# addtt/ladder-vae-pytorch

Hardware: AMD Instinct MI355X
Metric: training images/sec (ELBO step: fwd+bwd+Adamax) (higher is better)
Workload: dtype f32; 1 GPU; CIFAR10-shaped 15-layer LVAE (BASELINE configs[2]): 32x32x3, zdims 32x15, 4 blocks/layer, 64 filters, gated+skip, DMoL-10, dropout 0.2, free bits 1.0; batch_per_gpu=256, global_batch=256, parallelism=dp1, hip_graph=True

## Files before the change

### include/lvae_hip.h

```cpp
#ifndef LVAE_HIP_H
#define LVAE_HIP_H

#include <stddef.h>
#include <stdint.h>

#ifdef __cplusplus
extern "C" {
#endif

#define LVAE_ABI_VERSION 17

#define LVAE_EINVAL (-1)
#define LVAE_EALIGN (-2)
#define LVAE_EWORKSPACE (-3)

enum { LVAE_STATS_BN_FWD = 0, LVAE_STATS_BN_BWD = 1 };
enum { LVAE_PREC_F32 = 0, LVAE_PREC_BF16 = 1 };
enum { LVAE_DT_F32 = 0, LVAE_DT_BF16 = 1 };
enum {
  LVAE_FORM_AUTO = 0,
  LVAE_FORM_F32_MFMA = 1,
  LVAE_FORM_SIX_PRODUCT = 2,
  LVAE_FORM_SIX_PRODUCT_DIRECT = 3
};
// ... 96 lines not shown
  const float* dh;
  const float* x;
  const float* add;
  float* dgamma;
  float* dbeta;
  float* out;
  int32_t dh_bf16;
  int32_t reserved_;
  const float* drop;
} lvae_bn_apply;
size_t lvae_conv1x1_gate_bwd_wgrad_workspace(const lvae_conv_desc* d);
int32_t lvae_conv1x1_gate_bwd_wgrad_apply_ok(const lvae_conv_desc* d);
int lvae_conv1x1_gate_bwd_wgrad_f32(const lvae_conv_desc* d, const float* dout, const float* ab, const float* y, int32_t act,
                                    float* dw, int64_t dw_sk, int64_t dw_sn, float* db, void* workspace, size_t workspace_bytes,
                                    const lvae_bn_apply* ap, void* stream);

enum { LVAE_RB_PRO_AFFINE = 0, LVAE_RB_PRO_BN_APPLY = 1, LVAE_RB_PRO_GATE_BWD = 2 };
enum { LVAE_RB_EPI_PLAIN = 0, LVAE_RB_EPI_GATE = 1 };
typedef struct lvae_rb_ext {
  int32_t prologue, epilogue;
  const float* gate_w;
  int64_t gate_w_sk, gate_w_sn;
  void* gate_ws;
  int64_t gate_ws_bytes;
  int32_t gate_ws_ready;
  const float* gate_bias;
  int32_t act;
  const float* res;
  float* ab;
  float* out;
// ... 286 lines not shown
```

### ladder-vae-pytorch_amd/_C.py

```python
import ctypes as C
import os

import torch

_HERE = os.path.dirname(os.path.abspath(__file__))
LIB_PATH = os.path.join(_HERE, 'liblvae_hip.so')

ACT = {None: 0, 'none': 0, 'elu': 1, 'relu': 2, 'leakyrelu': 3, 'selu': 4}
GATHER_CONV, GATHER_TRANSPOSED = 0, 1
PREC_F32, PREC_BF16 = 0, 1
DT_F32, DT_BF16 = 0, 1
VARIANT_DIRECT, VARIANT_POS, VARIANT_WINO_F32, VARIANT_WINO_SIX, VARIANT_BF16_DIRECT, VARIANT_SIX_DIRECT = 0, 2, 3, 4, 5, 6
GATE_PERSISTENT, GATE_SINGLE_SHOT = 1, 2
WGRAD_VARIANT_GENERIC, WGRAD_VARIANT_IMG, WGRAD_VARIANT_BF16, WGRAD_VARIANT_WINO, WGRAD_VARIANT_DIRECT_1X1, WGRAD_VARIANT_TILE, WGRAD_VARIANT_THIN = range(7)
FEED_U8, FEED_F32 = 0, 1
FORM_AUTO, FORM_F32_MFMA, FORM_SIX_PRODUCT, FORM_SIX_PRODUCT_DIRECT = 0, 1, 2, 3


class LvaeHipError(RuntimeError):
    pass


class ConvDesc(C.Structure):
    _fields_ = [
# ... 82 lines not shown
    'lvae_conv2d_position_major': (_I, [C.POINTER(ConvDesc)]),
    'lvae_resblock_bf16_storage': (_I, [C.POINTER(ConvDesc)]),
    'lvae_conv2d_folds_bn_finalize': (_I, [C.POINTER(ConvDesc)]),
    'lvae_conv2d_stats_buffer_rows': (_I, [C.POINTER(ConvDesc)]),
    'lvae_conv2d_prepare_entry_bytes': (_Z, []),
    'lvae_conv2d_prepare_entry': (C.c_int, [C.POINTER(ConvDesc), _P]),
    'lvae_conv2d_prepare_weights': (C.c_int, [_P, _I, _I, _P]),
    'lvae_conv1x1_gate_f32': (C.c_int, [C.POINTER(ConvDesc), _P, _I, _P, _P]),
    'lvae_conv1x1_gate_stats_rows': (_I, [C.POINTER(ConvDesc)]),
    'lvae_conv1x1_gate_variant': (_I, [C.POINTER(ConvDesc)]),
    'lvae_conv1x1_gate_bwd_f32': (C.c_int, [C.POINTER(ConvDesc), _P, _P, _I, _P, _P]),
    'lvae_conv1x1_gate_bwd_ok': (_I, [C.POINTER(ConvDesc)]),
    'lvae_conv1x1_gate_bwd_wgrad_workspace': (_Z, [C.POINTER(ConvDesc)]),
    'lvae_conv1x1_gate_bwd_wgrad_apply_ok': (_I, [C.POINTER(ConvDesc)]),
    'lvae_conv1x1_gate_bwd_wgrad_f32': (C.c_int, [C.POINTER(ConvDesc), _P, _P, _P, _I, _P, _L, _L, _P, _P, _Z, C.POINTER(BnApply), _P]),
    'lvae_resblock_gate_workspace': (_Z, [C.POINTER(ConvDesc)]),
    'lvae_resblock_gate_prepare_entry': (C.c_int, [C.POINTER(ConvDesc), _P]),
    'lvae_resblock_conv_rows': (_I, [C.POINTER(ConvDesc)]),
    'lvae_resblock_conv_gate_rows': (_I, [C.POINTER(ConvDesc)]),
    'lvae_resblock_conv_workspace': (_Z, [C.POINTER(ConvDesc)]),
    'lvae_resblock_conv_prepare_entry': (C.c_int, [C.POINTER(ConvDesc), _P]),
    'lvae_resblock_conv_f32': (C.c_int, [C.POINTER(ConvDesc), C.POINTER(RbExt), _P]),
    'lvae_conv2d_wgrad_workspace': (_Z, [C.POINTER(ConvDesc)]),
    'lvae_conv2d_wgrad_f32': (C.c_int, [C.POINTER(ConvDesc), _P, _P, _P, _P, _Z, _P]),
    'lvae_conv2d_wgrad_bf16': (C.c_int, [C.POINTER(ConvDesc), _P, _P, _P, _P, _Z, _P]),
    'lvae_conv2d_wgrad_variant': (_I, [C.POINTER(ConvDesc)]),
    'lvae_conv2d_wgrad_apply_ok': (_I, [C.POINTER(ConvDesc)]),
    'lvae_conv2d_wgrad_apply_f32': (C.c_int, [C.POINTER(ConvDesc), C.POINTER(BnApply), _P, _P, _P, _Z, _P]),
    'lvae_conv2d_wgrad_pair_ok': (_I, [C.POINTER(ConvDesc), C.POINTER(ConvDesc)]),
    'lvae_conv2d_wgrad_pair_workspace': (_Z, [C.POINTER(ConvDesc), C.POINTER(ConvDesc)]),
# ... 141 lines not shown
```

### ladder-vae-pytorch_amd/csrc/conv1x1_gate_bwd_fused.hip

```cpp
#include "bf16_frag.h"
#include "bn_stats.h"
#include "lvae_host.h"

namespace lvae {

struct GbfArgs {
  const float* dout;
  const float* ab;
  const float* y;
  const float* w;
  int64_t w_sn;
  const float* drop;
  float* dx;
  float* slab_w;
  float* slab_b;
  int M, ohw, ntiles, act;
  int in_bf16, dx_bf16;
  lvae_bn_apply ap;
};

constexpr int GB_LDA = 132;
constexpr int GB_LDY = 68;

__global__ __launch_bounds__(512) void conv1x1_gate_bwd_fused_kernel(GbfArgs a) {
  kernarg_warmup<(sizeof(GbfArgs) < 1024 ? sizeof(GbfArgs) : 1024)>();
  extern __shared__ __attribute__((aligned(16))) float smem[];
  float* Bs = smem;
  float* As = Bs + 64 * GB_LDA;
  float* Ys = As + 64 * GB_LDA;
  const int t = threadIdx.x, lane = t & 63, wave = t >> 6;
  const bool wg_role = wave >= 4;
  const int wm = (wave & 3) >> 1, wn = wave & 1, li = lane & 31, lh = lane >> 5;
  const f32x4 zero4 = {0.f, 0.f, 0.f, 0.f};
// ... 110 lines not shown
    if (t < 128) {
      float v = 0.f;
#pragma unroll
      for (int g = 0; g < 32; ++g) v += red[g * 128 + t];
      a.slab_b[(size_t)blockIdx.x * 128 + t] = v;
    }
  }
}

constexpr int GBB_LDA = 136;
constexpr int GBB_LDY = 72;
constexpr size_t gbb_lds(int split) {
  return (size_t)split * (64 * GBB_LDA + 64 * GBB_LDY) * 2 + (size_t)64 * GB_LDY * 4 + 6 * 64 * 4 + (split == 3 ? (size_t)8 * 2 * 3 * 64 * 16 : 0);
}

template <int SPLIT, bool S16 = false, bool AP = false, bool ELU = false>
__global__ __launch_bounds__(512) void conv1x1_gate_bwd_fused_bf16_kernel(GbfArgs a) {
  kernarg_warmup<sizeof(GbfArgs)>();
#ifdef LVAE_GBF_DBG
  constexpr int dbg = LVAE_GBF_DBG;
#else
  constexpr int dbg = 0;
#endif
  const int gact = ELU ? LVAE_ACT_ELU : a.act, apact = ELU ? LVAE_ACT_ELU : a.ap.act;
  static_assert(SPLIT == 1 || !S16, "bf16 storage exists for the bf16-operand form only");
  extern __shared__ __attribute__((aligned(16))) unsigned char smem_raw[];
  constexpr int A_PLANE = 64 * GBB_LDA, Y_PLANE = 64 * GBB_LDY;
  __bf16* As = reinterpret_cast<__bf16*>(smem_raw);
  __bf16* Ys = As + SPLIT * A_PLANE;
  float* Os = reinterpret_cast<float*>(Ys + SPLIT * Y_PLANE);
  float* Cf = Os + 64 * GB_LDY;
  const int t = threadIdx.x, lane = t & 63, wave = t >> 6;
  const bool wg_role = wave >= 4;
  const int wm = (wave & 3) >> 1, wn = wave & 1, li = lane & 31, lh = lane >> 5, G = lane >> 4, i16 = lane & 15;
  const f32x4 zero4 = {0.f, 0.f, 0.f, 0.f};

  if (AP) {
    const int q = t & 31, rg = t >> 5, rows = a.ap.rows;
    f32x4 acc = zero4;
    for (int r = rg; r < rows; r += 16 * 8) {
// ... 65 lines not shown
  auto prefetch_row = [&](int tile, int u) {
    if (dbg & 1) {
      pg[u] = pa[u] = pb[u] = py[u] = zero4;
      if (AP) px[u] = pd[u] = zero4;
      return;
    }
    const int m = tile * 64 + r0 + 32 * u;
    const size_t mc = m < a.M ? (size_t)m : 0;
    if (AP) {
      pg[u] = load4_dt(a.ap.dh, mc * 64 + c4, ap_dh_bf);
      px[u] = *reinterpret_cast<const f32x4*>(a.ap.x + mc * 64 + c4);
      pd[u] = ap_add ? *reinterpret_cast<const f32x4*>(a.ap.add + mc * 64 + c4) : zero4;
    } else {
      pg[u] = *reinterpret_cast<const f32x4*>(a.dout + mc * 64 + c4);
    }
    pa[u] = load4_dt(a.ab, mc * 128 + c4, a.in_bf16 != 0);
    pb[u] = load4_dt(a.ab, mc * 128 + 64 + c4, a.in_bf16 != 0);
    py[u] = load4_dt(a.y, mc * 64 + c4, a.in_bf16 != 0);
  };
  auto prefetch = [&](int tile) {
    const int m0 = tile * 64;
    if (dbg & 1) {
      pg[0] = pg[1] = zero4;
#pragma unroll
      for (int u = 0; u < IT; ++u) pa[u] = pb[u] = py[u] = zero4;
#pragma unroll
      for (int u = 0; u < (AP ? 2 : 1); ++u) px[u] = pd[u] = zero4;
      qa = qb = qy = bf16x8{0, 0, 0, 0, 0, 0, 0, 0};
      return;
    }
    if (S16) {
      const int m = m0 + r8;
// ... 16 lines not shown
    }
#pragma unroll
    for (int u = 0; u < IT; ++u) prefetch_row(tile, u);
  };

  f32x16 accw[2];
#pragma unroll
  for (int j = 0; j < 2; ++j)
#pragma unroll
    for (int r = 0; r < 16; ++r) accw[j][r] = 0.f;
  f32x4 bs_lo = zero4, bs_hi = zero4;
  f32x4 bs_lo8 = zero4, bs_hi8 = zero4;
  const int trow = 8 * (G >> 1) + (i16 >> 2), tch = 16 * (G & 1) + 4 * (i16 & 3);
  using PO = PieceOrder<SPLIT>;

  int tile = blockIdx.x;
  if (tile < a.ntiles) prefetch(tile);
  for (; tile < a.ntiles; tile += gridDim.x) {
    const int m0 = tile * 64;
    if (S16) {
      f32x4 lo[2] = {zero4, zero4}, hi[2] = {zero4, zero4};
      bf16x8 yv = {0, 0, 0, 0, 0, 0, 0, 0};
      if (m0 + r8 < a.M) {
        if (AP) {
#pragma unroll
          for (int h = 0; h < 2; ++h) {
            pg[h] = ap_value(pg[h], px[h], pd[h], c8 + 4 * h);
            store_wt4(a.ap.out + (size_t)(m0 + r8) * 64 + c8 + 4 * h, pg[h]);
          }
        }
// ... 3 lines not shown
          for (int j = 0; j < 4; ++j) {
            const float av = (float)qa[4 * h + j], bv = (float)qb[4 * h + j];
            const float sg = sigmoidf_(bv);
            lo[h][j] = pg[h][j] * sg * act_grad(av, gact);
            hi[h][j] = pg[h][j] * act_fwd(av, gact) * sg * (1.f - sg);
          }
        yv = qy;
      }
      bs_lo += lo[0];
      bs_lo8 += lo[1];
      bs_hi += hi[0];
      bs_hi8 += hi[1];
      *reinterpret_cast<bf16x8*>(As + r8 * GBB_LDA + c8) = to_bf16x8(lo[0], lo[1]);
      *reinterpret_cast<bf16x8*>(As + r8 * GBB_LDA + 64 + c8) = to_bf16x8(hi[0], hi[1]);
      *reinterpret_cast<bf16x8*>(Ys + r8 * GBB_LDY + c8) = yv;
    } else
#pragma unroll
    for (int u = 0; u < IT; ++u) {
      const int r = r0 + 32 * u;
      f32x4 lo = zero4, hi = zero4, yv = zero4;
      if (m0 + r < a.M) {
        if (AP) {
          pg[u] = ap_value(pg[u], px[u], pd[u], c4);
          if (!(dbg & 4)) store_wt4(a.ap.out + (size_t)(m0 + r) * 64 + c4, pg[u]);
        }
        if (dbg & 8) {
          lo = pg[u] + pa[u];
          hi = pg[u] + pb[u];
        } else
#pragma unroll
        for (int j = 0; j < 4; ++j) {
// ... 2 lines not shown
          hi[j] = pg[u][j] * act_fwd(pa[u][j], gact) * sg * (1.f - sg);
        }
        yv = py[u];
      }
      bs_lo += lo;
      bs_hi += hi;
      if (tile + (int)gridDim.x < a.ntiles) prefetch_row(tile + gridDim.x, u);
      bf16x4 pl[SPLIT], ph[SPLIT], pyv[SPLIT];
      split4<SPLIT>(lo, pl);
      split4<SPLIT>(hi, ph);
      split4<SPLIT>(yv, pyv);
#pragma unroll
      for (int q = 0; q < SPLIT; ++q) {
        *reinterpret_cast<bf16x4*>(As + q * A_PLANE + r * GBB_LDA + c4) = pl[q];
        *reinterpret_cast<bf16x4*>(As + q * A_PLANE + r * GBB_LDA + 64 + c4) = ph[q];
        *reinterpret_cast<bf16x4*>(Ys + q * Y_PLANE + r * GBB_LDY + c4) = pyv[q];
      }
    }
    if (S16 && tile + (int)gridDim.x < a.ntiles) prefetch(tile + gridDim.x);
    lds_barrier();

    if (!wg_role) {
      f32x16 accx;
#pragma unroll
      for (int r = 0; r < 16; ++r) accx[r] = 0.f;
#pragma unroll
      for (int s = 0; s < 8; ++s) {
        bf16x8 af[SPLIT];
#pragma unroll
        for (int q = 0; q < SPLIT; ++q)
          af[q] = *reinterpret_cast<const bf16x8*>(As + q * A_PLANE + (wm * 32 + li) * GBB_LDA + 16 * s + 8 * lh);
        if (WLDS) {
// ... 103 lines not shown
  if (off || d == nullptr) return false;
  if (d->KH != 1 || d->KW != 1 || d->stride != 1 || d->pad != 0 || d->OH != d->H || d->OW != d->W) return false;
  if (d->C1 != 128 || d->C2 != 0 || d->Cout != 64 || d->w_sk != 1 || d->w_sn % 4 != 0 || d->in_scale != nullptr) return false;
  if (!al16_or_null(d->w) || !al16_or_null(d->y) || !al16_or_null(d->out_scale)) return false;
  const bool bf16 = d->precision == LVAE_PREC_BF16;
  if ((d->x_dtype == LVAE_DT_BF16 || d->y_dtype == LVAE_DT_BF16) && !bf16) return false;
  if (with_apply && d->form == LVAE_FORM_F32_MFMA && !bf16) return false;
  const int64_t M = (int64_t)d->N * d->H * d->W;
  static const int64_t min_m = tune("LVAE_GATE_FUSED_MIN_M", 256 * 64);
  if (M < min_m || M >= ((int64_t)1 << 31)) return false;
  p = ConvPlan{};
  p.workspace = (size_t)gbf_nwg(M) * (64 * 128 + 128) * sizeof(float);
  return true;
}

#define GBF_REQUIRE_AL16(p) LVAE_REQUIRE(al16_or_null(p), LVAE_EALIGN, "lvae_conv1x1_gate_bwd_wgrad_f32: " #p " must be 16-byte aligned")

static int conv1x1_gate_bwd_fused_launch(const lvae_conv_desc* d, const float* dout, const float* ab, const float* y, int act, float* dw,
                                         int64_t dw_sk, int64_t dw_sn, float* db, void* workspace, const lvae_bn_apply* ap, hipStream_t s) {
  GBF_REQUIRE_AL16(dout);
  GBF_REQUIRE_AL16(ab);
  GBF_REQUIRE_AL16(y);
  GBF_REQUIRE_AL16(workspace);
  GbfArgs a;
  a.ap = lvae_bn_apply{};
  if (ap != nullptr && ap->parts != nullptr) {
    GBF_REQUIRE_AL16(ap->parts);
    GBF_REQUIRE_AL16(ap->coef);
    GBF_REQUIRE_AL16(ap->dh);
    GBF_REQUIRE_AL16(ap->x);
    GBF_REQUIRE_AL16(ap->add);
    GBF_REQUIRE_AL16(ap->out);
    a.ap = *ap;
  }
  a.dout = dout;
  a.ab = ab;
  a.y = y;
  a.w = d->w;
  a.w_sn = d->w_sn;
// ... 19 lines not shown
  do {                                                                                                                                    \
    if (elu) hipLaunchKernelGGL((conv1x1_gate_bwd_fused_bf16_kernel<1, S16_, AP_, true>), grid, block, gbb_lds(1), s, a);                \
    else hipLaunchKernelGGL((conv1x1_gate_bwd_fused_bf16_kernel<1, S16_, AP_, false>), grid, block, gbb_lds(1), s, a);                   \
  } while (0)
    if (with_ap) {
      if (a.in_bf16 && a.dx_bf16) GBF_LAUNCH(true, true);
      else GBF_LAUNCH(false, true);
    } else if (a.in_bf16 && a.dx_bf16) GBF_LAUNCH(true, false);
    else GBF_LAUNCH(false, false);
#undef GBF_LAUNCH
    LVAE_LAUNCH_CHECK(name);
  } else {
    constexpr size_t lds3 = gbb_lds(3);
    int rc;
    if (f32_mfma) rc = launch_lds<conv1x1_gate_bwd_fused_kernel>(name, grid, block, lds, (int)lds, s, a);
    else if (with_ap && elu) rc = launch_lds<conv1x1_gate_bwd_fused_bf16_kernel<3, false, true, true>>(name, grid, block, lds3, (int)lds3, s, a);
    else if (with_ap) rc = launch_lds<conv1x1_gate_bwd_fused_bf16_kernel<3, false, true, false>>(name, grid, block, lds3, (int)lds3, s, a);
    else if (elu) rc = launch_lds<conv1x1_gate_bwd_fused_bf16_kernel<3, false, false, true>>(name, grid, block, lds3, (int)lds3, s, a);
    else rc = launch_lds<conv1x1_gate_bwd_fused_bf16_kernel<3, false, false, false>>(name, grid, block, lds3, (int)lds3, s, a);
    if (rc) return rc;
  }
  wgrad_reduce_launch(a.slab_w, a.slab_b, nwg, 1, 64, 128, 0, dw_sk, dw_sn, dw, db, s);
  LVAE_LAUNCH_CHECK("conv1x1_gate_bwd_fused_reduce");
  return 0;
}

}

using namespace lvae;

// ... 11 lines not shown
                                               float* dw, int64_t dw_sk, int64_t dw_sn, float* db, void* workspace,
                                               size_t workspace_bytes, const lvae_bn_apply* ap, void* stream) {
  const bool with_ap = ap != nullptr && ap->parts != nullptr;
  LVAE_REQUIRE(d && (dout || with_ap) && ab && y && d->y && dw && workspace, LVAE_EINVAL, "lvae_conv1x1_gate_bwd_wgrad_f32: null pointer");
  if (with_ap)
    LVAE_REQUIRE(ap->rows > 0 && ap->M == (int64_t)d->N * d->H * d->W && ap->coef && ap->dh && ap->x && ap->out, LVAE_EINVAL,
                 "lvae_conv1x1_gate_bwd_wgrad_f32: deferred apply needs parts / rows, M = N*H*W, the coefficient block, dh, x and out");
  ConvPlan p;
  LVAE_REQUIRE(conv1x1_gate_bwd_fused_plan(d, with_ap, p), LVAE_EINVAL,
               "lvae_conv1x1_gate_bwd_wgrad_f32: not supported (needs the gate of a 64-channel block: 1x1, 128 -> 64 dgrad view, at least 16384 "
               "pixels, 16-byte aligned w / y / out_scale, bf16 storage only with precision LVAE_PREC_BF16, a deferred apply not with "
               "LVAE_FORM_F32_MFMA); use lvae_conv1x1_gate_bwd_f32 + lvae_conv2d_wgrad_f32");
  LVAE_REQUIRE(workspace_bytes >= p.workspace, LVAE_EWORKSPACE, "lvae_conv1x1_gate_bwd_wgrad_f32: workspace %zu < %zu", workspace_bytes, p.workspace);
  return conv1x1_gate_bwd_fused_launch(d, dout, ab, y, act, dw, dw_sk, dw_sn, db, workspace, ap, (hipStream_t)stream);
}
```

### ladder-vae-pytorch_amd/kernels.py

```python
import ctypes as C
import weakref

import torch

from . import _C
from ._C import ACT, BnFold, ConvDesc, RbExt, GATHER_CONV, GATHER_TRANSPOSED, PREC_BF16, PREC_F32, call, ptr, ptr_dt, stream_ptr

_ws_cache = {}

precision = PREC_F32


form = _C.FORM_AUTO


class use_form:
    def __init__(self, f):
        self.f = f

    def __enter__(self):
        global form
        self.prev, form = form, self.f

    def __exit__(self, *exc):
# ... 317 lines not shown
    d = _desc(g, weight, ab, None, N, H, W, H, W, g.Cin, g.s_co, g.s_ci, GATHER_TRANSPOSED, out_scale=out_scale, y=dx)
    lib = _C.load()
    need = lib.lvae_conv1x1_gate_bwd_wgrad_workspace(C.byref(d))
    if not need or (apply is not None and not lib.lvae_conv1x1_gate_bwd_wgrad_apply_ok(C.byref(d))):
        return None
    ws = workspace(need, dout.device)
    ap = None
    if apply is not None:
        ap = _C.BnApply(ptr(apply.parts), apply.parts.shape[0], ACT[apply.act], N * H * W, ptr(apply.coef0), ptr_dt(apply.dh), ptr(apply.x),
                        ptr(apply.add), ptr(apply.dgamma), ptr(apply.dbeta), ptr(apply.out), int(apply.dh.dtype == torch.bfloat16), 0)
    call('lvae_conv1x1_gate_bwd_wgrad_f32', C.byref(d), ptr(dout), ptr_dt(ab), ptr_dt(y), ACT[act], ptr(dweight), g.s_ci, g.s_co, ptr(dbias),
         ws.data_ptr(), ws.numel(), C.byref(ap) if ap is not None else None, stream_ptr())
    return dx


def _rb_desc(x_like, weight, g, dgrad, y=None, bias=None, in_scale=None, in_shift=None, in_act=None, out_scale=None):
    N, H, W, _ = x_like.shape
    if dgrad:
        d = _desc(g, weight, x_like, None, N, H, W, H, W, g.Cin, g.s_co, g.s_ci, GATHER_TRANSPOSED, out_scale=out_scale, y=y)
    else:
        d = _desc(g, weight, x_like, None, N, H, W, H, W, g.Cout, g.s_ci, g.s_co, GATHER_CONV, bias, in_scale, in_shift, in_act, out_scale, None, y)
    need = _C.load().lvae_resblock_conv_workspace(C.byref(d))
    if need:
        prepared.attach(d, weight, x_like.device, need, 'lvae_resblock_conv_prepare_entry')
    return d, need


def _rb_gate_ws(e, gate_w, gate_g, device, bwd):
    gd = ConvDesc()
    gd.w, gd.precision = ptr(gate_w), precision
# ... 74 lines not shown
    return y, parts, coef


def rb_gate_rows(x, weight, g, whole_image=True):
    d = _rb_query_desc(x, weight, g)
    if d is None:
        return 0
    rows = int(_C.load().lvae_resblock_conv_rows(C.byref(d)))
    if rows > 0:
        return rows if whole_image else 0
    _conv_ws(d, weight, x.device)
    return int(_C.load().lvae_resblock_conv_gate_rows(C.byref(d)))


def rb_conv_gate(x, weight, g, bias, in_act, out_scale, gate_w, gate_g, gate_bias, res, act, in_bn=None, coef=None, stats_pivot=None,
                 prefetch=None):
    N, H, W, _ = x.shape
    dev = x.device
    y = torch.empty((N, H, W, g.Cout), dtype=torch.float32, device=dev)
    ab = torch.empty((N, H, W, gate_g.Cout), dtype=torch.float32, device=dev)
    out = torch.empty((N, H, W, gate_g.Cout // 2), dtype=torch.float32, device=dev)
    d, need = _rb_desc(x, weight, g, False, y, bias, None, None, in_act, out_scale)
    can_fold = True
    if not need:
        _conv_ws(d, weight, dev)
        can_fold = bool(_C.load().lvae_conv2d_folds_bn_finalize(C.byref(d)))
    coef, keep = _in_bn(d, in_bn, x, can_fold, coef)
    e = RbExt()
    e.prologue, e.epilogue = _C.RB_PRO_AFFINE, _C.RB_EPI_GATE
    _rb_gate_ws(e, gate_w, gate_g, dev, False)
    e.gate_bias, e.act = ptr(gate_bias), ACT[act]
    e.res, e.ab, e.out = ptr(res), ptr(ab), ptr(out)
    parts = None
    if stats_pivot is not None:
        rows = _C.load().lvae_resblock_conv_gate_rows(C.byref(d))
        buf = torch.empty((rows + 1, 2, g.Cout), dtype=torch.float32, device=dev)
        parts = StatParts(buf, rows, True)
# ... 1062 lines not shown
```

### ladder-vae-pytorch_amd/ops.py

```python
from types import SimpleNamespace

import torch
from torch.autograd import Function

from . import kernels as K
from . import resblock as RB

_const_cache = {}


def _ones_zeros(C, device):
    key = (C, device)
    if key not in _const_cache:
        _const_cache[key] = (torch.ones(C, device=device), torch.zeros(C, device=device))
    return _const_cache[key]


def grad_buf(p):
    if not p.requires_grad:
        return None
    if p.grad is None:
        p.grad = torch.zeros_like(p)
    return p.grad

# ... 125 lines not shown

def _fwd_fused_gate(call, x, blk, m1, m2, training):
    act, st, bn2, cv1, cv2, gate = blk.act, blk.sched, blk.bn2, blk.conv1, blk.conv2, blk.gate
    whole = call.plan.forward == 'whole-image'
    if whole:
        in_bn, coef1 = _bn_of_half(x, blk.bn1, True, call.parts, call.pivot)
        st.link('fwd', K.rb_weight_ranges(x, cv1.weight, cv1.geom(), False))
        y1, parts2, coef1 = K.rb_conv(x, cv1.weight, cv1.geom(), cv1.bias, act, m1, in_bn=in_bn, coef=coef1, stats_pivot=bn2.running_mean,
                                      prefetch=K.rb_weight_ranges(x, cv2.weight, cv2.geom(), False, gate=(gate.weight, gate.geom())))
    else:
        y1, parts2, coef1 = _conv_half(x, blk.bn1, cv1, act, m1, True, call.parts, call.pivot, bn2.running_mean, False)
    in_bn, coef2 = _bn_of_half(y1, bn2, True, parts2, bn2.running_mean)
    call.out_pivot = coef1[2].detach() if call.plan.gate_stats else None
    y2, ab, out, call.out_parts, coef2 = K.rb_conv_gate(y1, cv2.weight, cv2.geom(), cv2.bias, act, m2, gate.weight, gate.geom(), gate.bias, x, act,
                                                        in_bn=in_bn, coef=coef2, stats_pivot=call.out_pivot,
                                                        prefetch=st.next_ranges('fwd') if whole else None)
    return y1, y2, ab, out, coef1, coef2


def _fwd_per_op(call, x, blk, m1, m2, training):
    act, bn2, gate, s16 = blk.act, blk.bn2, blk.gate, call.plan.bf16_internals
    want_stats = training and bn2 is not None and bn2.running_mean is not None
    y1, parts2, coef1 = _conv_half(x, blk.bn1, blk.conv1, act, m1, training, call.parts, call.pivot, bn2.running_mean if want_stats else None, s16)
    y2, _, coef2 = _conv_half(y1, bn2, blk.conv2, act, m2, training, parts2, bn2.running_mean if bn2 is not None else None, None, s16)
    if gate is None:
        return y1, y2, None, K.add(y2, x), coef1, coef2
    call.out_pivot = coef1[2].detach() if call.plan.gate_stats else None
    r = K.conv1x1_gate(y2, gate.weight, gate.geom(), gate.bias, x, act, stats_pivot=call.out_pivot)
    ab, out, call.out_parts = r if call.out_pivot is not None else r + (None,)
    return y1, y2, ab, out, coef1, coef2

# ... 56 lines not shown
    if gw.requires_grad:
        wgrad(y2, dab, gw, gate.geom(), grad_buf(gw), grad_buf(gate.bias))
    wgrad(y1, dy2, w2, cv2.geom(), grad_buf(w2), grad_buf(cv2.bias), in_scale=coef2[0], in_shift=coef2[1], in_act=act)
    dy1, dh1, parts1 = K.rb_apply_dgrad(parts2, dh2, y1, coef2[0], act, grad_buf(bn2.weight), grad_buf(bn2.bias), m1, w1, cv1.geom(),
                                        bn_bwd=(x, coef1[0], act), prefetch=st.next_ranges('bwd'))
    wgrad(x, dy1, w1, cv1.geom(), grad_buf(w1), grad_buf(cv1.bias), in_scale=coef1[0], in_shift=coef1[1], in_act=act)
    return dh1, parts1


def _bwd_gate(blk, plan, dout, y2, ab, m2):
    gate, act, s16 = blk.gate, blk.act, plan.bf16_internals
    if gate is None:
        return K.scale_rows_add(dout, m2, None) if m2 is not None else dout
    gw = gate.weight
    if plan.backward == 'persistent-gate':
        dy2 = K.conv1x1_gate_bwd_wgrad(dout, ab, y2, gw, gate.geom(), act, grad_buf(gw), grad_buf(gate.bias), out_scale=m2, out_bf16=s16,
                                       apply=blk.sched.take_pending(dout))
        if dy2 is None:
            raise K._C.LvaeHipError("residual block: the persistent gate backward the block was planned with did not take this shape")
        return dy2
    if s16:
        raise K._C.LvaeHipError("bf16-stored residual block: the fused gate backward did not take this shape")
    dab, dy2 = K.conv1x1_gate_bwd(dout, ab, gw, gate.geom(), act, out_scale=m2)
    wgrad(y2, dab, gw, gate.geom(), grad_buf(gw), grad_buf(gate.bias))
    return dy2


def _bwd_half(ctx, cv, bn, h, dy, coef, wgrad_done=False):
    w, g, act = cv.weight, cv.geom(), ctx.blk.act
    if not wgrad_done:
        wgrad(h, dy, w, g, grad_buf(w), grad_buf(cv.bias), in_scale=coef[0], in_shift=coef[1], in_act=act)
    if bn is not None and ctx.training and K.bn_coef_block(*coef):
# ... 502 lines not shown
```

### ladder-vae-pytorch_amd/resblock.py

```python
import os
import weakref
from typing import NamedTuple, Optional

import torch

from . import kernels as K


class Switches:

    def __init__(self, env):
        on = lambda name: env.get(name, '1') != '0'
        self.wgrad_flush = int(env.get('LVAE_WGRAD_FLUSH', '1024'))
        self.dgrad_cat = on('LVAE_DGRAD_CAT')
        self.wgrad_apply = on('LVAE_WGRAD_APPLY')
        self.wgrad_apply_maxw = int(env.get('LVAE_WGRAD_APPLY_MAXW', '16'))
        self.wgrad_pair = on('LVAE_WGRAD_PAIR')
        self.wgrad_pair_maxw = int(env.get('LVAE_WGRAD_PAIR_MAXW', '16'))
        self.gate_stats = env.get('LVAE_NO_GATE_STATS') is None
        self.defer_apply = on('LVAE_DEFER_APPLY')
        self.defer_apply_large = on('LVAE_DEFER_APPLY_LARGE')
        self.rb_fwd_min_hw, self.rb_bwd_min_hw = int(env.get('LVAE_RB_FWD_MIN_HW', '16')), int(env.get('LVAE_RB_BWD_MIN_HW', '1'))
        self.rb_gate_large = on('LVAE_RB_GATE_LARGE')
        self.stoch_block = on('LVAE_STOCH_BLOCK')
        self.stoch_block_bwd = on('LVAE_STOCH_BLOCK_BWD')


switches = Switches(os.environ)


class BlockPlan(NamedTuple):
    forward: str
    bf16_internals: bool
    gate_stats: bool
    backward: Optional[str]
    wgrad_absorbs_apply: bool
    wgrad_pair: bool
    accepts: Optional[str]


def plan_block(blk, x, training):
    sw, grad = switches, torch.is_grad_enabled()
    cv1, cv2, gate, bn1, bn2 = blk.conv1, blk.conv2, blk.gate, blk.bn1, blk.bn2
    gated_bn = gate is not None and bn1 is not None and bn2 is not None and gate.bias is not None
    full = (training and gated_bn and cv1.bias is not None and cv2.bias is not None and bn1.running_mean is not None and
            bn2.running_mean is not None and x.dtype == torch.float32)
    hw = x.shape[1] * x.shape[2]
    whole = full and K.rb_rows(x, cv1.weight, cv1.geom()) > 0
    whole_fwd, whole_bwd = whole and 0 < sw.rb_fwd_min_hw <= hw, whole and 0 < sw.rb_bwd_min_hw <= hw
    s16 = bool(not whole_fwd and not whole_bwd and gated_bn and K.resblock_bf16_storage(x, cv1.weight, cv1.geom()))
    if whole_fwd:
        forward = 'whole-image'
    elif full and not s16 and sw.rb_gate_large and K.rb_gate_rows(x, cv2.weight, cv2.geom(), whole_image=False) > 0:
# ... 3 lines not shown
    gate_stats = gate is not None and training and bn1 is not None and bn1.running_mean is not None and sw.gate_stats
    backward, accepts, absorbs, pair = None, None, False, False
    if grad and whole_bwd:
        backward, accepts = 'whole-image', 'f32-dh'
    elif grad:
        backward = 'composed'
        if gate is not None and gate.bias is not None and gate.weight.requires_grad and \
                K.gate_bwd_fused_ws(x, gate.weight, gate.geom(), gate.weight.grad) > 0:
            backward = 'persistent-gate'
            if training and not whole_fwd and sw.defer_apply_large and K.gate_bwd_apply_ok(x, gate.weight, gate.geom(), gate.weight.grad):
                accepts = 'any-dh'
        absorbs = bool(training and bn2 is not None and sw.wgrad_apply and not s16 and cv1.weight.requires_grad and
                       x.shape[2] <= sw.wgrad_apply_maxw and K.conv2d_wgrad_apply_ok(x, cv1.weight, cv1.geom()))
        pair = bool(absorbs and sw.wgrad_pair and cv2.weight.requires_grad and x.shape[2] <= sw.wgrad_pair_maxw and
                    K.conv2d_wgrad_pair_ok(x, cv1.weight, cv1.geom(), x, cv2.weight, cv2.geom()))
    return BlockPlan(forward, s16, gate_stats, backward, absorbs, pair, accepts)


class Handover(NamedTuple):
    parts: object
    pivot: object
    producer: object = None
    accepts: Optional[str] = None


def passed_on(src, aliases):
    h = getattr(src, '_lvae_handover', None)
    if h is not None and h.parts is not None:
        for a in aliases:
            a._lvae_handover = Handover(h.parts, h.pivot)

# ... 47 lines not shown
```

Measured before the change: 9216 images/s.

## Recompute gate pre-activations in backward instead of storing them in forward

Adds a recompute variant of the fused persistent gate backward kernel. It rebuilds the 1x1 gate pre-activations (ab) from y2 using a six-product bf16 MFMA against the prepared gate weight planes plus bias, rather than reading ab saved by the forward pass. The forward wino-gate path then skips allocating and writing ab. The aim is to cut the HBM write and read of the 128-channel ab tensor on small-resolution blocks (width at most 16 by default). The cost is an extra GEMM and extra LDS round-trips with barriers inside the backward kernel, plus possibly a weight-plane prepare when the planes are not ready.

After: 9356 images/s, median of 6. +1.5%, better.

```diff
diff --git a/include/lvae_hip.h b/include/lvae_hip.h
--- a/include/lvae_hip.h
+++ b/include/lvae_hip.h
@@ -134,6 +134,11 @@
 int lvae_conv1x1_gate_bwd_wgrad_f32(const lvae_conv_desc* d, const float* dout, const float* ab, const float* y, int32_t act,
                                     float* dw, int64_t dw_sk, int64_t dw_sn, float* db, void* workspace, size_t workspace_bytes,
                                     const lvae_bn_apply* ap, void* stream);
+int32_t lvae_conv1x1_gate_bwd_wgrad_recompute_ok(const lvae_conv_desc* d);
+int lvae_conv1x1_gate_bwd_wgrad_recompute_f32(const lvae_conv_desc* d, const float* dout, const float* y, int32_t act, void* gate_ws,
+                                              int64_t gate_ws_bytes, int32_t gate_ws_ready, const float* gate_w, int64_t gate_w_sk,
+                                              int64_t gate_w_sn, const float* gate_bias, float* dw, int64_t dw_sk, int64_t dw_sn,
+                                              float* db, void* workspace, size_t workspace_bytes, const lvae_bn_apply* ap, void* stream);
 
 enum { LVAE_RB_PRO_AFFINE = 0, LVAE_RB_PRO_BN_APPLY = 1, LVAE_RB_PRO_GATE_BWD = 2 };
 enum { LVAE_RB_EPI_PLAIN = 0, LVAE_RB_EPI_GATE = 1 };
diff --git a/ladder-vae-pytorch_amd/_C.py b/ladder-vae-pytorch_amd/_C.py
--- a/ladder-vae-pytorch_amd/_C.py
+++ b/ladder-vae-pytorch_amd/_C.py
@@ -120,6 +120,9 @@
     'lvae_conv1x1_gate_bwd_wgrad_workspace': (_Z, [C.POINTER(ConvDesc)]),
     'lvae_conv1x1_gate_bwd_wgrad_apply_ok': (_I, [C.POINTER(ConvDesc)]),
     'lvae_conv1x1_gate_bwd_wgrad_f32': (C.c_int, [C.POINTER(ConvDesc), _P, _P, _P, _I, _P, _L, _L, _P, _P, _Z, C.POINTER(BnApply), _P]),
+    'lvae_conv1x1_gate_bwd_wgrad_recompute_ok': (_I, [C.POINTER(ConvDesc)]),
+    'lvae_conv1x1_gate_bwd_wgrad_recompute_f32': (C.c_int, [C.POINTER(ConvDesc), _P, _P, _I, _P, _L, _I, _P, _L, _L, _P, _P, _L, _L, _P, _P, _Z,
+                                                            C.POINTER(BnApply), _P]),
     'lvae_resblock_gate_workspace': (_Z, [C.POINTER(ConvDesc)]),
     'lvae_resblock_gate_prepare_entry': (C.c_int, [C.POINTER(ConvDesc), _P]),
     'lvae_resblock_conv_rows': (_I, [C.POINTER(ConvDesc)]),
diff --git a/ladder-vae-pytorch_amd/csrc/conv1x1_gate_bwd_fused.hip b/ladder-vae-pytorch_amd/csrc/conv1x1_gate_bwd_fused.hip
--- a/ladder-vae-pytorch_amd/csrc/conv1x1_gate_bwd_fused.hip
+++ b/ladder-vae-pytorch_amd/csrc/conv1x1_gate_bwd_fused.hip
@@ -17,6 +17,8 @@
   int M, ohw, ntiles, act;
   int in_bf16, dx_bf16;
   lvae_bn_apply ap;
+  const __bf16* gws;
+  const float* gbias;
 };
 
 constexpr int GB_LDA = 132;
@@ -157,7 +159,7 @@
   return (size_t)split * (64 * GBB_LDA + 64 * GBB_LDY) * 2 + (size_t)64 * GB_LDY * 4 + 6 * 64 * 4 + (split == 3 ? (size_t)8 * 2 * 3 * 64 * 16 : 0);
 }
 
-template <int SPLIT, bool S16 = false, bool AP = false, bool ELU = false>
+template <int SPLIT, bool S16 = false, bool AP = false, bool ELU = false, bool RC = false>
 __global__ __launch_bounds__(512) void conv1x1_gate_bwd_fused_bf16_kernel(GbfArgs a) {
   kernarg_warmup<sizeof(GbfArgs)>();
 #ifdef LVAE_GBF_DBG
@@ -167,6 +169,7 @@
 #endif
   const int gact = ELU ? LVAE_ACT_ELU : a.act, apact = ELU ? LVAE_ACT_ELU : a.ap.act;
   static_assert(SPLIT == 1 || !S16, "bf16 storage exists for the bf16-operand form only");
+  static_assert(!RC || (SPLIT == 3 && !S16), "the recomputed pre-activations exist in the six-product form only");
   extern __shared__ __attribute__((aligned(16))) unsigned char smem_raw[];
   constexpr int A_PLANE = 64 * GBB_LDA, Y_PLANE = 64 * GBB_LDY;
   __bf16* As = reinterpret_cast<__bf16*>(smem_raw);
@@ -262,8 +265,10 @@
     } else {
       pg[u] = *reinterpret_cast<const f32x4*>(a.dout + mc * 64 + c4);
     }
-    pa[u] = load4_dt(a.ab, mc * 128 + c4, a.in_bf16 != 0);
-    pb[u] = load4_dt(a.ab, mc * 128 + 64 + c4, a.in_bf16 != 0);
+    if (!RC) {
+      pa[u] = load4_dt(a.ab, mc * 128 + c4, a.in_bf16 != 0);
+      pb[u] = load4_dt(a.ab, mc * 128 + 64 + c4, a.in_bf16 != 0);
+    }
     py[u] = load4_dt(a.y, mc * 64 + c4, a.in_bf16 != 0);
   };
   auto prefetch = [&](int tile) {
@@ -310,6 +315,21 @@
   const int trow = 8 * (G >> 1) + (i16 >> 2), tch = 16 * (G & 1) + 4 * (i16 & 3);
   using PO = PieceOrder<SPLIT>;
 
+  const int rrb = wave >> 2, rct = wave & 3;
+  bf16x8 gq[RC ? 4 : 1][SPLIT];
+  f32x4 gba = zero4, gbb = zero4;
+  if (RC) {
+    const __bf16* gws = a.gws + lane * 8;
+#pragma unroll
+    for (int s4 = 0; s4 < 4; ++s4)
+#pragma unroll
+      for (int q = 0; q < SPLIT; ++q) gq[s4][q] = *reinterpret_cast<const bf16x8*>(gws + ((size_t)(s4 * 4 + rct) * SPLIT + q) * 512);
+    if (a.gbias) {
+      gba = *reinterpret_cast<const f32x4*>(a.gbias + c4);
+      gbb = *reinterpret_cast<const f32x4*>(a.gbias + 64 + c4);
+    }
+  }
+
   int tile = blockIdx.x;
   if (tile < a.ntiles) prefetch(tile);
   for (; tile < a.ntiles; tile += gridDim.x) {
@@ -343,7 +363,49 @@
       *reinterpret_cast<bf16x8*>(As + r8 * GBB_LDA + c8) = to_bf16x8(lo[0], lo[1]);
       *reinterpret_cast<bf16x8*>(As + r8 * GBB_LDA + 64 + c8) = to_bf16x8(hi[0], hi[1]);
       *reinterpret_cast<bf16x8*>(Ys + r8 * GBB_LDY + c8) = yv;
-    } else
+    } else {
+    if (RC) {
+#pragma unroll
+      for (int u = 0; u < IT; ++u) {
+        const int r = r0 + 32 * u;
+        bf16x4 pyv[SPLIT];
+        split4<SPLIT>(m0 + r < a.M ? py[u] : zero4, pyv);
+#pragma unroll
+        for (int q = 0; q < SPLIT; ++q) *reinterpret_cast<bf16x4*>(Ys + q * Y_PLANE + r * GBB_LDY + c4) = pyv[q];
+      }
+      lds_barrier();
+      f32x16 accq;
+#pragma unroll
+      for (int r = 0; r < 16; ++r) accq[r] = 0.f;
+#pragma unroll
+      for (int s4 = 0; s4 < 4; ++s4) {
+        bf16x8 af[SPLIT];
+#pragma unroll
+        for (int q = 0; q < SPLIT; ++q)
+          af[q] = *reinterpret_cast<const bf16x8*>(Ys + q * Y_PLANE + (rrb * 32 + li) * GBB_LDY + 16 * s4 + 8 * lh);
+#pragma unroll
+        for (int k = 0; k < PO::N; ++k) { if (dbg & 16) accq[k] += (float)af[PO::A[k]][0] * (float)gq[RC ? s4 : 0][PO::B[k]][1]; else accq = __builtin_amdgcn_mfma_f32_32x32x16_bf16(af[PO::A[k]], gq[RC ? s4 : 0][PO::B[k]], accq, 0, 0, 0); }
+      }
+      if (dbg & 32) {
+#pragma unroll
+        for (int u = 0; u < IT; ++u) {
+          pa[u] = gba + accq[u];
+          pb[u] = gbb + accq[2 + u];
+        }
+      } else {
+      float* Qs = reinterpret_cast<float*>(As);
+#pragma unroll
+      for (int r = 0; r < 16; ++r) Qs[(rrb * 32 + (r & 3) + 8 * (r >> 2) + 4 * lh) * GB_LDA + rct * 32 + li] = accq[r];
+      lds_barrier();
+#pragma unroll
+      for (int u = 0; u < IT; ++u) {
+        const int r = r0 + 32 * u;
+        pa[u] = *reinterpret_cast<const f32x4*>(Qs + r * GB_LDA + c4) + gba;
+        pb[u] = *reinterpret_cast<const f32x4*>(Qs + r * GB_LDA + 64 + c4) + gbb;
+      }
+      lds_barrier();
+      }
+    }
 #pragma unroll
     for (int u = 0; u < IT; ++u) {
       const int r = r0 + 32 * u;
@@ -376,8 +438,9 @@
       for (int q = 0; q < SPLIT; ++q) {
         *reinterpret_cast<bf16x4*>(As + q * A_PLANE + r * GBB_LDA + c4) = pl[q];
         *reinterpret_cast<bf16x4*>(As + q * A_PLANE + r * GBB_LDA + 64 + c4) = ph[q];
-        *reinterpret_cast<bf16x4*>(Ys + q * Y_PLANE + r * GBB_LDY + c4) = pyv[q];
-      }
+        if (!RC) *reinterpret_cast<bf16x4*>(Ys + q * Y_PLANE + r * GBB_LDY + c4) = pyv[q];
+      }
+    }
     }
     if (S16 && tile + (int)gridDim.x < a.ntiles) prefetch(tile + gridDim.x);
     lds_barrier();
@@ -511,15 +574,33 @@
   return true;
 }
 
+static bool gbf_recompute_plan(const lvae_conv_desc* d, bool with_apply, ConvPlan& p) {
+  static const bool off = tune("LVAE_DISABLE_GATE_RECOMPUTE", 0) != 0;
+  if (off || !conv1x1_gate_bwd_fused_plan(d, with_apply, p)) return false;
+  return d->precision == LVAE_PREC_F32 && d->form != LVAE_FORM_F32_MFMA && d->x_dtype != LVAE_DT_BF16 && d->y_dtype != LVAE_DT_BF16;
+}
+static size_t gbf_planes_bytes() {
+  lvae_conv_desc g = lvae_conv_desc{};
+  g.C1 = 64;
+  g.Cout = 128;
+  return resblock_gate_ws_bytes(&g, 3);
+}
+
 #define GBF_REQUIRE_AL16(p) LVAE_REQUIRE(al16_or_null(p), LVAE_EALIGN, "lvae_conv1x1_gate_bwd_wgrad_f32: " #p " must be 16-byte aligned")
 
 static int conv1x1_gate_bwd_fused_launch(const lvae_conv_desc* d, const float* dout, const float* ab, const float* y, int act, float* dw,
-                                         int64_t dw_sk, int64_t dw_sn, float* db, void* workspace, const lvae_bn_apply* ap, hipStream_t s) {
+                                         int64_t dw_sk, int64_t dw_sn, float* db, void* workspace, const lvae_bn_apply* ap, hipStream_t s,
+                                         const void* gws = nullptr, const float* gbias = nullptr) {
   GBF_REQUIRE_AL16(dout);
   GBF_REQUIRE_AL16(ab);
   GBF_REQUIRE_AL16(y);
   GBF_REQUIRE_AL16(workspace);
+  GBF_REQUIRE_AL16(gws);
+  GBF_REQUIRE_AL16(gbias);
+  const bool rcp = ab == nullptr;
   GbfArgs a;
+  a.gws = static_cast<const __bf16*>(gws);
+  a.gbias = gbias;
   a.ap = lvae_bn_apply{};
   if (ap != nullptr && ap->parts != nullptr) {
     GBF_REQUIRE_AL16(ap->parts);
@@ -569,6 +650,10 @@
     constexpr size_t lds3 = gbb_lds(3);
     int rc;
     if (f32_mfma) rc = launch_lds<conv1x1_gate_bwd_fused_kernel>(name, grid, block, lds, (int)lds, s, a);
+    else if (rcp && with_ap && elu) rc = launch_lds<conv1x1_gate_bwd_fused_bf16_kernel<3, false, true, true, true>>(name, grid, block, lds3, (int)lds3, s, a);
+    else if (rcp && with_ap) rc = launch_lds<conv1x1_gate_bwd_fused_bf16_kernel<3, false, true, false, true>>(name, grid, block, lds3, (int)lds3, s, a);
+    else if (rcp && elu) rc = launch_lds<conv1x1_gate_bwd_fused_bf16_kernel<3, false, false, true, true>>(name, grid, block, lds3, (int)lds3, s, a);
+    else if (rcp) rc = launch_lds<conv1x1_gate_bwd_fused_bf16_kernel<3, false, false, false, true>>(name, grid, block, lds3, (int)lds3, s, a);
     else if (with_ap && elu) rc = launch_lds<conv1x1_gate_bwd_fused_bf16_kernel<3, false, true, true>>(name, grid, block, lds3, (int)lds3, s, a);
     else if (with_ap) rc = launch_lds<conv1x1_gate_bwd_fused_bf16_kernel<3, false, true, false>>(name, grid, block, lds3, (int)lds3, s, a);
     else if (elu) rc = launch_lds<conv1x1_gate_bwd_fused_bf16_kernel<3, false, false, true>>(name, grid, block, lds3, (int)lds3, s, a);
@@ -610,3 +695,37 @@
   LVAE_REQUIRE(workspace_bytes >= p.workspace, LVAE_EWORKSPACE, "lvae_conv1x1_gate_bwd_wgrad_f32: workspace %zu < %zu", workspace_bytes, p.workspace);
   return conv1x1_gate_bwd_fused_launch(d, dout, ab, y, act, dw, dw_sk, dw_sn, db, workspace, ap, (hipStream_t)stream);
 }
+
+extern "C" int32_t lvae_conv1x1_gate_bwd_wgrad_recompute_ok(const lvae_conv_desc* d) {
+  ConvPlan p;
+  return gbf_recompute_plan(d, false, p) && gbf_recompute_plan(d, true, p) ? 1 : 0;
+}
+
+extern "C" int lvae_conv1x1_gate_bwd_wgrad_recompute_f32(const lvae_conv_desc* d, const float* dout, const float* y, int32_t act, void* gate_ws,
+                                                         int64_t gate_ws_bytes, int32_t gate_ws_ready, const float* gate_w, int64_t gate_w_sk,
+                                                         int64_t gate_w_sn, const float* gate_bias, float* dw, int64_t dw_sk, int64_t dw_sn,
+                                                         float* db, void* workspace, size_t workspace_bytes, const lvae_bn_apply* ap,
+                                                         void* stream) {
+  const char* who = "lvae_conv1x1_gate_bwd_wgrad_recompute_f32";
+  const bool with_ap = ap != nullptr && ap->parts != nullptr;
+  LVAE_REQUIRE(d && (dout || with_ap) && y && d->y && dw && workspace, LVAE_EINVAL, "%s: null pointer", who);
+  if (with_ap)
+    LVAE_REQUIRE(ap->rows > 0 && ap->M == (int64_t)d->N * d->H * d->W && ap->coef && ap->dh && ap->x && ap->out, LVAE_EINVAL,
+                 "%s: deferred apply needs parts / rows, M = N*H*W, the coefficient block, dh, x and out", who);
+  ConvPlan p;
+  LVAE_REQUIRE(gbf_recompute_plan(d, with_ap, p), LVAE_EINVAL,
+               "%s: not supported (needs what lvae_conv1x1_gate_bwd_wgrad_f32 needs, fp32 tensors, precision LVAE_PREC_F32 and not "
+               "LVAE_FORM_F32_MFMA: lvae_conv1x1_gate_bwd_wgrad_recompute_ok)", who);
+  LVAE_REQUIRE(workspace_bytes >= p.workspace, LVAE_EWORKSPACE, "%s: workspace %zu < %zu", who, workspace_bytes, p.workspace);
+  LVAE_REQUIRE(gate_ws != nullptr && al16_or_null(gate_ws) && gate_ws_bytes >= 0 && (size_t)gate_ws_bytes >= gbf_planes_bytes() &&
+                   (gate_ws_ready || gate_w != nullptr),
+               LVAE_EWORKSPACE, "%s: gate_ws missing or smaller than lvae_resblock_gate_workspace() of the forward gate, or not ready and no gate_w", who);
+  if (!gate_ws_ready) {
+    lvae_conv_desc g = lvae_conv_desc{};
+    g.w = gate_w; g.w_sk = gate_w_sk; g.w_sn = gate_w_sn; g.precision = LVAE_PREC_F32; g.C1 = 64; g.Cout = 128;
+    g.workspace = gate_ws; g.workspace_bytes = gate_ws_bytes;
+    const int rc = resblock_gate_prepare_single(&g, 3, (hipStream_t)stream);
+    if (rc) return rc;
+  }
+  return conv1x1_gate_bwd_fused_launch(d, dout, nullptr, y, act, dw, dw_sk, dw_sn, db, workspace, ap, (hipStream_t)stream, gate_ws, gate_bias);
+}
diff --git a/ladder-vae-pytorch_amd/kernels.py b/ladder-vae-pytorch_amd/kernels.py
--- a/ladder-vae-pytorch_amd/kernels.py
+++ b/ladder-vae-pytorch_amd/kernels.py
@@ -355,6 +355,36 @@
     return dx
 
 
+def gate_bwd_recompute_ok(x_like, weight, g, dweight=None):
+    d = _gate_bwd_fused_desc(x_like, weight, g, dweight)
+    return d is not None and x_like.dtype == torch.float32 and bool(_C.load().lvae_conv1x1_gate_bwd_wgrad_recompute_ok(C.byref(d)))
+
+
+def conv1x1_gate_bwd_wgrad_recompute(dout, y, weight, g, bias, act, dweight, dbias, out_scale=None, apply=None):
+    _chk_nhwc(dout, 'dout')
+    N, H, W, Cn = dout.shape
+    if g.Cout != 2 * Cn or tuple(dweight.stride()) != tuple(weight.stride()) or y.dtype != torch.float32:
+        return None
+    dx = torch.empty((N, H, W, g.Cin), dtype=torch.float32, device=dout.device)
+    d = _desc(g, weight, y, None, N, H, W, H, W, g.Cin, g.s_co, g.s_ci, GATHER_TRANSPOSED, out_scale=out_scale, y=dx)
+    d.C1 = g.Cout
+    lib = _C.load()
+    need = lib.lvae_conv1x1_gate_bwd_wgrad_workspace(C.byref(d))
+    if not need or not lib.lvae_conv1x1_gate_bwd_wgrad_recompute_ok(C.byref(d)):
+        return None
+    e = RbExt()
+    _rb_gate_ws(e, weight, g, dout.device, False)
+    ws = workspace(need, dout.device)
+    ap = None
+    if apply is not None:
+        ap = _C.BnApply(ptr(apply.parts), apply.parts.shape[0], ACT[apply.act], N * H * W, ptr(apply.coef0), ptr_dt(apply.dh), ptr(apply.x),
+                        ptr(apply.add), ptr(apply.dgamma), ptr(apply.dbeta), ptr(apply.out), int(apply.dh.dtype == torch.bfloat16), 0)
+    call('lvae_conv1x1_gate_bwd_wgrad_recompute_f32', C.byref(d), ptr(dout), ptr(y), ACT[act], e.gate_ws, e.gate_ws_bytes, e.gate_ws_ready,
+         e.gate_w, e.gate_w_sk, e.gate_w_sn, ptr(bias), ptr(dweight), g.s_ci, g.s_co, ptr(dbias), ws.data_ptr(), ws.numel(),
+         C.byref(ap) if ap is not None else None, stream_ptr())
+    return dx
+
+
 def _rb_desc(x_like, weight, g, dgrad, y=None, bias=None, in_scale=None, in_shift=None, in_act=None, out_scale=None):
     N, H, W, _ = x_like.shape
     if dgrad:
@@ -459,13 +489,15 @@
 
 
 def rb_conv_gate(x, weight, g, bias, in_act, out_scale, gate_w, gate_g, gate_bias, res, act, in_bn=None, coef=None, stats_pivot=None,
-                 prefetch=None):
+                 prefetch=None, want_ab=True):
     N, H, W, _ = x.shape
     dev = x.device
     y = torch.empty((N, H, W, g.Cout), dtype=torch.float32, device=dev)
-    ab = torch.empty((N, H, W, gate_g.Cout), dtype=torch.float32, device=dev)
     out = torch.empty((N, H, W, gate_g.Cout // 2), dtype=torch.float32, device=dev)
     d, need = _rb_desc(x, weight, g, False, y, bias, None, None, in_act, out_scale)
+    if need and not want_ab:
+        raise _C.LvaeHipError("rb_conv_gate: the whole-image kernels always store ab")
+    ab = torch.empty((N, H, W, gate_g.Cout), dtype=torch.float32, device=dev) if want_ab else None
     can_fold = True
     if not need:
         _conv_ws(d, weight, dev)
diff --git a/ladder-vae-pytorch_amd/ops.py b/ladder-vae-pytorch_amd/ops.py
--- a/ladder-vae-pytorch_amd/ops.py
+++ b/ladder-vae-pytorch_amd/ops.py
@@ -163,7 +163,8 @@
     call.out_pivot = coef1[2].detach() if call.plan.gate_stats else None
     y2, ab, out, call.out_parts, coef2 = K.rb_conv_gate(y1, cv2.weight, cv2.geom(), cv2.bias, act, m2, gate.weight, gate.geom(), gate.bias, x, act,
                                                         in_bn=in_bn, coef=coef2, stats_pivot=call.out_pivot,
-                                                        prefetch=st.next_ranges('fwd') if whole else None)
+                                                        prefetch=st.next_ranges('fwd') if whole else None,
+                                                        want_ab=not call.plan.recompute_ab)
     return y1, y2, ab, out, coef1, coef2
 
 
@@ -250,8 +251,12 @@
         return K.scale_rows_add(dout, m2, None) if m2 is not None else dout
     gw = gate.weight
     if plan.backward == 'persistent-gate':
-        dy2 = K.conv1x1_gate_bwd_wgrad(dout, ab, y2, gw, gate.geom(), act, grad_buf(gw), grad_buf(gate.bias), out_scale=m2, out_bf16=s16,
-                                       apply=blk.sched.take_pending(dout))
+        if plan.recompute_ab:
+            dy2 = K.conv1x1_gate_bwd_wgrad_recompute(dout, y2, gw, gate.geom(), gate.bias, act, grad_buf(gw), grad_buf(gate.bias), out_scale=m2,
+                                                     apply=blk.sched.take_pending(dout))
+        else:
+            dy2 = K.conv1x1_gate_bwd_wgrad(dout, ab, y2, gw, gate.geom(), act, grad_buf(gw), grad_buf(gate.bias), out_scale=m2, out_bf16=s16,
+                                           apply=blk.sched.take_pending(dout))
         if dy2 is None:
             raise K._C.LvaeHipError("residual block: the persistent gate backward the block was planned with did not take this shape")
         return dy2
diff --git a/ladder-vae-pytorch_amd/resblock.py b/ladder-vae-pytorch_amd/resblock.py
--- a/ladder-vae-pytorch_amd/resblock.py
+++ b/ladder-vae-pytorch_amd/resblock.py
@@ -24,6 +24,8 @@
         self.rb_gate_large = on('LVAE_RB_GATE_LARGE')
         self.stoch_block = on('LVAE_STOCH_BLOCK')
         self.stoch_block_bwd = on('LVAE_STOCH_BLOCK_BWD')
+        self.gate_recompute = on('LVAE_GATE_RECOMPUTE')
+        self.gate_recompute_maxw = int(env.get('LVAE_GATE_RECOMPUTE_MAXW', '16'))
 
 
 switches = Switches(os.environ)
@@ -37,6 +39,7 @@
     wgrad_absorbs_apply: bool
     wgrad_pair: bool
     accepts: Optional[str]
+    recompute_ab: bool = False
 
 
 def plan_block(blk, x, training):
@@ -70,7 +73,9 @@
                        x.shape[2] <= sw.wgrad_apply_maxw and K.conv2d_wgrad_apply_ok(x, cv1.weight, cv1.geom()))
         pair = bool(absorbs and sw.wgrad_pair and cv2.weight.requires_grad and x.shape[2] <= sw.wgrad_pair_maxw and
                     K.conv2d_wgrad_pair_ok(x, cv1.weight, cv1.geom(), x, cv2.weight, cv2.geom()))
-    return BlockPlan(forward, s16, gate_stats, backward, absorbs, pair, accepts)
+    recompute = bool(forward == 'wino-gate' and backward == 'persistent-gate' and not s16 and sw.gate_recompute and
+                     x.shape[2] <= sw.gate_recompute_maxw and K.gate_bwd_recompute_ok(x, gate.weight, gate.geom(), gate.weight.grad))
+    return BlockPlan(forward, s16, gate_stats, backward, absorbs, pair, accepts, recompute)
 
 
 class Handover(NamedTuple):
```
